# andimarafioti/faster-qwen3-tts

Measured on AMD Instinct MI355X. Metric: real-time factor (audio s / wall s), Qwen3-TTS-12Hz-0.6B voice-clone streaming chunk_size=8; p50 TTFA in ttfa_ms_p50, higher is better.
Workload: dtype bf16

## Files before the change

faster-qwen3-tts_amd/csrc/decode_kernels.cuh:

```cuda
#pragma once
#include "fq3_common.cuh"

namespace fq3 {

enum { PRO_PLAIN = 0, PRO_NORM = 1, PRO_COMBINE = 2 };
enum { EPI_STORE = 0, EPI_RESIDUAL = 1, EPI_SWIGLU = 2 };

constexpr int kHeadDim = 128;
constexpr int kKeysPerTile = 64;
constexpr int kMaxWorkers = 8;
constexpr int kPartStride = kHeadDim + 4;


struct GemvArgs {
    const void* W; int N; int K;
    const void* x;
    const void* norm_w; float eps;
    const void* bias;
    void* y;
    const void* res;
    void* xn_out;
    int up_off;
    const float* part; int n_part; int rep;
    const void* x2; void* y2; const void* res2; size_t part_stride2;
// ... 371 lines not shown
        for (int w = 0; w < 4; ++w) {
            const float ww = __expf(wm[w][h] - M);
            num = fmaf(ww, wo[w][h][d], num);
            den = fmaf(ww, wl[w][h], den);
        }
        float* p = a.part + (((size_t)g * kMaxWorkers + s) * REP + h) * kPartStride;
        p[d] = num;
        if (d == 0) { p[HD] = M; p[HD + 1] = den; }
    }
}

template <typename T, int REP, bool PAGED>
__global__ __launch_bounds__(256) void attn_decode_kernel(AttnArgs a) { attn_decode_body<T, REP, PAGED>(a); }

template <typename T>
__device__ __forceinline__ void attn_pred_body(const AttnArgs& a, int head) {
    constexpr int HD = kHeadDim;
    const int g = head / a.rep, hh = head - g * a.rep;
    const int lane = threadIdx.x & 63, sub = lane >> 4, c = lane & 15;
    const int pos = a.pos_imm;
    const T* qkv = reinterpret_cast<const T*>(a.qkv);
    const int q_dim = a.n_kv * a.rep * HD, kv_dim = a.n_kv * HD;
    T* kc = reinterpret_cast<T*>(a.kcache) + (size_t)g * a.max_seq * HD;
    T* vc = reinterpret_cast<T*>(a.vcache) + (size_t)g * a.max_seq * HD;
    Raw8<T> qraw, knraw, vnraw, qwraw, kwraw, kr[4], vr[4];
    ldraw<false>(qraw, qkv + (size_t)head * HD + c * 8);
    ldraw<false>(knraw, qkv + q_dim + (size_t)g * HD + c * 8);
    ldraw<false>(vnraw, qkv + q_dim + kv_dim + (size_t)g * HD + c * 8);
    ldraw<false>(qwraw, reinterpret_cast<const T*>(a.q_norm_w) + c * 8);
    ldraw<false>(kwraw, reinterpret_cast<const T*>(a.k_norm_w) + c * 8);
    const f32x4 cs0 = *reinterpret_cast<const f32x4*>(a.cos_row + ((c * 8) & 63)), cs1 = *reinterpret_cast<const f32x4*>(a.cos_row + ((c * 8 + 4) & 63));
    const f32x4 sn0 = *reinterpret_cast<const f32x4*>(a.sin_row + ((c * 8) & 63)), sn1 = *reinterpret_cast<const f32x4*>(a.sin_row + ((c * 8 + 4) & 63));
#pragma unroll
    for (int i = 0; i < 4; ++i) {
        int key = i * 4 + sub;
        key = key < a.max_seq ? key : a.max_seq - 1;
        ldraw<false>(kr[i], kc + (size_t)key * HD + c * 8);
        ldraw<false>(vr[i], vc + (size_t)key * HD + c * 8);
    }
    __builtin_amdgcn_sched_barrier(0);
    const float sgn = c < 8 ? -1.f : 1.f;
    const float cs[8] = {cs0.x, cs0.y, cs0.z, cs0.w, cs1.x, cs1.y, cs1.z, cs1.w};
    const float sn[8] = {sgn * sn0.x, sgn * sn0.y, sgn * sn0.z, sgn * sn0.w, sgn * sn1.x, sgn * sn1.y, sgn * sn1.z, sgn * sn1.w};
    auto norm_rope = [&](const Raw8<T>& raw, const Raw8<T>& wraw, float (&out)[8]) {
        float x[8], w[8];
        unpack(raw, x); unpack(wraw, w);
        float ss = 0.f;
#pragma unroll
        for (int i = 0; i < 8; ++i) ss = fmaf(x[i], x[i], ss);
        ss = row16_sum(ss);
        const float rs = 1.0f / sqrtf(ss / (float)HD + a.eps);
#pragma unroll
        for (int i = 0; i < 8; i += 2) {
            float u = x[i] * rs, v = x[i + 1] * rs;
            DT<T>::rnd2(u, v);
            u *= w[i]; v *= w[i + 1];
            DT<T>::rnd2(u, v);
            x[i] = u; x[i + 1] = v;
        }
#pragma unroll
        for (int i = 0; i < 8; i += 2) {
            float a0 = x[i] * cs[i], a1 = x[i + 1] * cs[i + 1];
            float b0 = row16_xor8(x[i]) * sn[i], b1 = row16_xor8(x[i + 1]) * sn[i + 1];
            DT<T>::rnd2(a0, a1); DT<T>::rnd2(b0, b1);
            float r0 = a0 + b0, r1 = a1 + b1;
            DT<T>::rnd2(r0, r1);
            out[i] = r0; out[i + 1] = r1;
        }
    };
    float qr[8], knew[8], vnew[8];
    norm_rope(qraw, qwraw, qr);
    norm_rope(knraw, kwraw, knew);
    unpack(vnraw, vnew);
    if (hh == 0 && sub == 0) {
        DT<T>::st8(kc + (size_t)pos * HD + c * 8, knew);
        DT<T>::st8(vc + (size_t)pos * HD + c * 8, vnew);
    }
    float sc[5];
#pragma unroll
    for (int i = 0; i < 4; ++i) {
        float kf[8], s = 0.f;
        unpack(kr[i], kf);
#pragma unroll
        for (int d = 0; d < 8; ++d) s = fmaf(qr[d], kf[d], s);
// ... 18 lines not shown
    for (int i = 0; i < 4; ++i) {
        float vf[8];
        if (!(i * 4 + sub < pos)) zero(vr[i]);
        unpack(vr[i], vf);
#pragma unroll
        for (int d = 0; d < 8; ++d) o[d] = fmaf(p[i], vf[d], o[d]);
    }
    const float inv = 1.0f / lsum;
#pragma unroll
    for (int d = 0; d < 8; ++d) o[d] = xrow_sum(o[d]) * inv;
    if (sub == 0) DT<T>::st8(reinterpret_cast<T*>(a.out) + (size_t)head * HD + c * 8, o);
}

template <typename T>
__device__ __forceinline__ void attn_pred_body(const AttnArgs& a) { attn_pred_body<T>(a, (int)blockIdx.x); }

template <typename T, int REP>
__device__ __forceinline__ void attn_pred_group_body(const AttnArgs& a, int g) {
    constexpr int HD = kHeadDim;
    const int lane = threadIdx.x & 63, sub = lane >> 4, c = lane & 15;
    const int pos = a.pos_imm;
    const T* qkv = reinterpret_cast<const T*>(a.qkv);
    const int q_dim = a.n_kv * REP * HD, kv_dim = a.n_kv * HD;
    T* kc = reinterpret_cast<T*>(a.kcache) + (size_t)g * a.max_seq * HD;
    T* vc = reinterpret_cast<T*>(a.vcache) + (size_t)g * a.max_seq * HD;
    Raw8<T> qraw[REP], knraw, vnraw, qwraw, kwraw, kr[4], vr[4];
#pragma unroll
    for (int h = 0; h < REP; ++h) ldraw<false>(qraw[h], qkv + (size_t)(g * REP + h) * HD + c * 8);
    ldraw<false>(knraw, qkv + q_dim + (size_t)g * HD + c * 8);
    ldraw<false>(vnraw, qkv + q_dim + kv_dim + (size_t)g * HD + c * 8);
    ldraw<false>(qwraw, reinterpret_cast<const T*>(a.q_norm_w) + c * 8);
    ldraw<false>(kwraw, reinterpret_cast<const T*>(a.k_norm_w) + c * 8);
    const f32x4 cs0 = *reinterpret_cast<const f32x4*>(a.cos_row + ((c * 8) & 63)), cs1 = *reinterpret_cast<const f32x4*>(a.cos_row + ((c * 8 + 4) & 63));
    const f32x4 sn0 = *reinterpret_cast<const f32x4*>(a.sin_row + ((c * 8) & 63)), sn1 = *reinterpret_cast<const f32x4*>(a.sin_row + ((c * 8 + 4) & 63));
#pragma unroll
    for (int i = 0; i < 4; ++i) {
        int key = i * 4 + sub;
        key = key < pos ? key : 0;
        ldraw<false>(kr[i], kc + (size_t)key * HD + c * 8);
        ldraw<false>(vr[i], vc + (size_t)key * HD + c * 8);
    }
    __builtin_amdgcn_sched_barrier(0);
    const float sgn = c < 8 ? -1.f : 1.f;
    const float cs[8] = {cs0.x, cs0.y, cs0.z, cs0.w, cs1.x, cs1.y, cs1.z, cs1.w};
    const float sn[8] = {sgn * sn0.x, sgn * sn0.y, sgn * sn0.z, sgn * sn0.w, sgn * sn1.x, sgn * sn1.y, sgn * sn1.z, sgn * sn1.w};
    auto norm_rope = [&](const Raw8<T>& raw, const Raw8<T>& wraw, float (&out)[8]) {
        float x[8], w[8];
        unpack(raw, x); unpack(wraw, w);
        float ss = 0.f;
#pragma unroll
        for (int i = 0; i < 8; ++i) ss = fmaf(x[i], x[i], ss);
        ss = row16_sum(ss);
        const float rs = 1.0f / sqrtf(ss / (float)HD + a.eps);
#pragma unroll
        for (int i = 0; i < 8; i += 2) {
            float u = x[i] * rs, v = x[i + 1] * rs;
            DT<T>::rnd2(u, v);
            u *= w[i]; v *= w[i + 1];
            DT<T>::rnd2(u, v);
            x[i] = u; x[i + 1] = v;
        }
#pragma unroll
        for (int i = 0; i < 8; i += 2) {
            float a0 = x[i] * cs[i], a1 = x[i + 1] * cs[i + 1];
            float b0 = row16_xor8(x[i]) * sn[i], b1 = row16_xor8(x[i + 1]) * sn[i + 1];
            DT<T>::rnd2(a0, a1); DT<T>::rnd2(b0, b1);
            float r0 = a0 + b0, r1 = a1 + b1;
            DT<T>::rnd2(r0, r1);
            out[i] = r0; out[i + 1] = r1;
        }
    };
    float knew[8], vnew[8];
    norm_rope(knraw, kwraw, knew);
    unpack(vnraw, vnew);
    if (sub == 0) {
        DT<T>::st8(kc + (size_t)pos * HD + c * 8, knew);
        DT<T>::st8(vc + (size_t)pos * HD + c * 8, vnew);
    }
    float kf[4][8], vf[4][8];
#pragma unroll
    for (int i = 0; i < 4; ++i) {
        unpack(kr[i], kf[i]);
        if (!(i * 4 + sub < pos)) zero(vr[i]);
        unpack(vr[i], vf[i]);
    }
#pragma unroll
    for (int h = 0; h < REP; ++h) {
        float qr[8];
        norm_rope(qraw[h], qwraw, qr);
        float sc[5];
#pragma unroll
        for (int i = 0; i < 4; ++i) {
            float s = 0.f;
#pragma unroll
            for (int d = 0; d < 8; ++d) s = fmaf(qr[d], kf[i][d], s);
            s = row16_sum(s);
            sc[i] = (i * 4 + sub < pos) ? s * a.scale : -INFINITY;
        }
        {
            float s = 0.f;
#pragma unroll
            for (int d = 0; d < 8; ++d) s = fmaf(qr[d], knew[d], s);
            s = row16_sum(s);
            sc[4] = sub == 0 ? s * a.scale : -INFINITY;
        }
        const float mx = wave_max(fmaxf(fmaxf(fmaxf(sc[0], sc[1]), fmaxf(sc[2], sc[3])), sc[4]));
        float p[5], lsum = 0.f, o[8];
#pragma unroll
        for (int i = 0; i < 5; ++i) { p[i] = __expf(sc[i] - mx); lsum += p[i]; }
        lsum = wave_sum(lsum) * (1.0f / 16.0f);
#pragma unroll
        for (int d = 0; d < 8; ++d) o[d] = p[4] * vnew[d];
#pragma unroll
        for (int i = 0; i < 4; ++i)
#pragma unroll
            for (int d = 0; d < 8; ++d) o[d] = fmaf(p[i], vf[i][d], o[d]);
        const float inv = 1.0f / lsum;
#pragma unroll
        for (int d = 0; d < 8; ++d) o[d] = xrow_sum(o[d]) * inv;
        if (sub == 0) DT<T>::st8(reinterpret_cast<T*>(a.out) + (size_t)(g * REP + h) * HD + c * 8, o);
    }
}

template <typename T>
__global__ __launch_bounds__(64) void attn_pred_kernel(AttnArgs a) { attn_pred_body<T>(a); }

template <typename T>
__global__ __launch_bounds__(256) void rmsnorm_kernel(const T* x, const T* w, T* y, int K, float eps) {
    __shared__ float red[8];
    float ss = 0.f;
    for (int e = threadIdx.x; e < K; e += 256) { const float v = DT<T>::ld(x + e); ss = fmaf(v, v, ss); }
    ss = block_sum<4>(ss, red);
    const float rs = 1.0f / sqrtf(ss / (float)K + eps);
    for (int e = threadIdx.x; e < K; e += 256)
        DT<T>::st(y + e, DT<T>::ld(w + e) * DT<T>::rnd(DT<T>::ld(x + e) * rs));
}

template <typename T>
__global__ void copy_kernel(T* dst, const T* src, int n) {
    const int i = blockIdx.x * blockDim.x + threadIdx.x;
// ... 97 lines not shown
```

faster-qwen3-tts_amd/csrc/fq3_api.hip:

```cpp
#define FQ3_SKINNY_EXTERN
#include "fq3_ctx.h"
#include "sampler.cuh"
#include "sampler_wave.cuh"
#include "skinny_gemm.cuh"

#include <cstdio>
#include <cstdlib>
#include <cstring>
#include <map>
#include <string>
#include <type_traits>
#include <vector>

using namespace fq3;

static thread_local std::string g_err;
static int fail(int code, const std::string& m) { g_err = m; return code; }
int fq3_fail_(int code, const std::string& m) { return fail(code, m); }
#define HIPCHK(x) do { hipError_t e_ = (x); if (e_ != hipSuccess) return fail(FQ3_EHIP, std::string(#x) + ": " + hipGetErrorString(e_)); } while (0)

extern "C" const char* fq3_last_error(void) { return g_err.c_str(); }
extern "C" void fq3_set_error_(const char* msg) { g_err = msg ? msg : ""; }
extern "C" int fq3_abi_version(void) { return FQ3_ABI_VERSION; }

// ... 217 lines not shown
}

extern "C" int fq3_set_option(fq3_ctx* c, const char* key, int value) {
    if (!c || !key) return fail(FQ3_EINVAL, "null argument");
    const std::string k(key);
    if (k == "weight_nt") c->opt_nt = value;
    else if (k == "pred_m2") c->opt_m2 = value;
    else if (k == "pred_attn") c->opt_pred_attn = value;
    else if (k == "rows_per_wave_max") c->opt_rmax = value;
    else if (k == "prefill_mode") c->prefill_mode = value;
    else if (k == "flash_prefill") c->opt_flash_prefill = value;
    else if (k == "flash_small") c->opt_flash_small = value;
    else if (k == "swiglu_tile") c->opt_swiglu_tile = value;
    else if (k == "packed_weights") c->opt_packed = value;
    else if (k == "skinny_gemm") c->opt_no_skinny = !value;
    else return fail(FQ3_EINVAL, "unknown option: " + k);
    fq3_graph_reset(c);
    return FQ3_OK;
}

extern "C" int fq3_graph_reset(fq3_ctx* c) {
    if (!c) return fail(FQ3_EINVAL, "null ctx");
    if (c->exec) { (void)hipGraphExecDestroy(c->exec); c->exec = nullptr; }
    if (c->graph) { (void)hipGraphDestroy(c->graph); c->graph = nullptr; }
    return FQ3_OK;
}

namespace {
struct PackedEntry { void* p; int refs; int N, K; };
std::mutex g_packed_mu;
// ... 44 lines not shown
            if (int r = take(l.o, d.hidden, qd, 0)) return r;
            if (int r = take(l.gate_up, 2 * d.inter, d.hidden, 1)) return r;
            if (int r = take(l.gate_up, 2 * d.inter, d.hidden, 0)) return r;
            if (int r = take(l.down, d.hidden, d.inter, 0)) return r;
        }
        return FQ3_OK;
    };
    if (int r = stack(c->tl, c->cfg.talker)) return r;
    if (int r = stack(c->pl, c->cfg.predictor)) return r;
    for (const fq3_layer_weights& l : c->tl) if (int r = take(l.gate_up, 2 * c->cfg.talker.inter, c->cfg.talker.hidden, 2)) return r;
    if (int r = take(c->wt.codec_head, c->cfg.talker.vocab, c->cfg.talker.hidden, 0)) return r;
    for (const void* h : c->lmh) if (int r = take(h, c->cfg.predictor.vocab, c->cfg.predictor.hidden, 0)) return r;
    return FQ3_OK;
}

extern "C" int fq3_ctx_destroy(fq3_ctx* c) {
    if (!c) return FQ3_OK;
    (void)hipDeviceSynchronize();
    fq3_graph_reset(c);
    packed_release_all(c);
    if (c->cap_stream) (void)hipStreamDestroy(c->cap_stream);
    if (fq3_kv_pool* p = c->tk.pool) {
        (void)fq3_kv_release(c, 0);
        bool last;
        { std::lock_guard<std::mutex> lk(p->mu); last = --p->users == 0; }
        if (p->is_private && last) pool_free_(p);
    }
    for (void* p : c->allocs) (void)hipFree(p);
    delete c;
    return FQ3_OK;
}

extern "C" int fq3_bind_weights(fq3_ctx* c, const fq3_weight_table* w) {
    if (!c || !w) return fail(FQ3_EINVAL, "null argument");
    const int G = c->cfg.num_code_groups;
// ... 4 lines not shown
    if (c->cfg.has_projection && !w->proj_w) return fail(FQ3_EINVAL, "has_projection set but proj_w is null");
    if (w->talker_rope_len < c->cfg.max_seq_len || w->pred_rope_len < G + 1)
        return fail(FQ3_EINVAL, "rope tables shorter than the caches");
    c->wt = *w;
    c->tl.assign(w->talker_layers, w->talker_layers + c->cfg.talker.n_layers);
    c->pl.assign(w->predictor_layers, w->predictor_layers + c->cfg.predictor.n_layers);
    c->pemb.assign(w->predictor_embeddings, w->predictor_embeddings + (G - 1));
    c->lmh.assign(w->lm_heads, w->lm_heads + (G - 1));
    for (auto& l : c->tl) if (!l.qkv || !l.o || !l.gate_up || !l.down || !l.input_norm || !l.post_norm || !l.q_norm || !l.k_norm)
        return fail(FQ3_EINVAL, "talker layer has null weights");
    for (auto& l : c->pl) if (!l.qkv || !l.o || !l.gate_up || !l.down || !l.input_norm || !l.post_norm || !l.q_norm || !l.k_norm)
        return fail(FQ3_EINVAL, "predictor layer has null weights");
    HIPCHK(hipMemcpy(c->d_pemb, c->pemb.data(), (G - 1) * sizeof(void*), hipMemcpyHostToDevice));
    (void)hipDeviceSynchronize();
    packed_release_all(c);
    if (int r = packed_acquire_all(c)) { packed_release_all(c); return r; }
    c->bound = true;
    fq3_graph_reset(c);
    return FQ3_OK;
}

static thread_local int g_rmax = 2;
template <typename T, int NCH, int PRO, int EPI, bool NT, int M = 1>
static void launch_gemv_n(const GemvArgs& a, hipStream_t s) {
    const int rmax = g_rmax;
    int R = (a.N + 1023) / 1024;
    if (R > MaxRows<NCH, EPI>::v) R = MaxRows<NCH, EPI>::v;
    if (rmax > 0 && R > rmax) R = rmax;
    if (R < 1) R = 1;
    const int grid = (a.N + 4 * R - 1) / (4 * R);
    const size_t shm = PRO == PRO_COMBINE ? (size_t)M * a.K * sizeof(float) : 0;
// ... 37 lines not shown
    return nt ? launch_gemv_t<float, PRO, EPI, true>(a, s) : launch_gemv_t<float, PRO, EPI, false>(a, s);
}

template <typename T, bool PAGED>
static void launch_attn_p(const AttnArgs& a, int rep, int workers, hipStream_t s) {
    dim3 grid(a.n_kv, workers);
    if (rep == 1) hipLaunchKernelGGL((attn_decode_kernel<T, 1, PAGED>), grid, dim3(256), 0, s, a);
    else if (rep == 2) hipLaunchKernelGGL((attn_decode_kernel<T, 2, PAGED>), grid, dim3(256), 0, s, a);
    else hipLaunchKernelGGL((attn_decode_kernel<T, 4, PAGED>), grid, dim3(256), 0, s, a);
}
template <typename T>
static void launch_attn_t(const AttnArgs& a, int rep, int workers, hipStream_t s) {
    if (a.table) launch_attn_p<T, true>(a, rep, workers, s); else launch_attn_p<T, false>(a, rep, workers, s);
}

struct StepSrc { const void* x0; const int* pos_ptr; int pos_imm; bool kv_only_tail = false; };

static int run_stack(fq3_ctx* c, bool talker, const StepSrc& src, hipStream_t s) {
    const fq3_stack_dims& d = talker ? c->cfg.talker : c->cfg.predictor;
    const std::vector<fq3_layer_weights>& L = talker ? c->tl : c->pl;
    StackBufs& kv = talker ? c->tk : c->pk;
    const int rep = d.n_heads / d.n_kv_heads;
    const int q_dim = d.n_heads * kHeadDim, kv_dim = d.n_kv_heads * kHeadDim;
    const bool nt = c->opt_nt == 2 || (c->opt_nt == 1 && talker);
    const float *cos_row, *sin_row;
    if (src.pos_ptr) { cos_row = c->rope_now; sin_row = c->rope_now + 64; }
    else {
        const int rl = talker ? c->wt.talker_rope_len : c->wt.pred_rope_len;
        int rp = src.pos_imm + (talker ? c->rope_delta : 0);
        rp = rp < 0 ? 0 : (rp >= rl ? rl - 1 : rp);
        cos_row = (talker ? c->wt.talker_cos : c->wt.pred_cos) + (size_t)rp * 64;
        sin_row = (talker ? c->wt.talker_sin : c->wt.pred_sin) + (size_t)rp * 64;
    }
    for (int i = 0; i < d.n_layers; ++i) {
        const fq3_layer_weights& w = L[i];
        const void* xin = i == 0 ? src.x0 : c->h;
        GemvArgs g{};
        g.eps = d.rms_eps;
        g.W = w.qkv; g.N = q_dim + 2 * kv_dim; g.K = d.hidden; g.x = xin;
        g.norm_w = w.input_norm; g.y = c->qkv;
        if (int r = launch_gemv<PRO_NORM, EPI_STORE>(c, g, nt, s)) return r;
        const bool tail_skip = src.kv_only_tail && i == d.n_layers - 1;
        GemvArgs o{};
        o.W = w.o; o.N = d.hidden; o.K = q_dim; o.y = c->h; o.res = xin; o.rep = rep;
        AttnArgs a{};
        a.qkv = c->qkv; a.q_norm_w = w.q_norm; a.k_norm_w = w.k_norm; a.eps = d.rms_eps;
        a.cos_row = cos_row; a.sin_row = sin_row;
        a.kcache = kv.k[i]; a.vcache = kv.v[i]; a.max_seq = kv.max_seq;
        a.table = kv.d_table; a.blk_stride = kv.pool ? (int)kv.pool->blk_elems : 0;
        a.pos_ptr = src.pos_ptr; a.pos_imm = src.pos_imm;
        a.done_ptr = src.pos_ptr ? &c->st->done : nullptr;
        a.n_pad = talker ? c->n_pad : 0;
        a.n_kv = d.n_kv_heads; a.part = c->part;
        a.scale = 1.0f / sqrtf((float)kHeadDim);
        a.rep = rep; a.out = c->attn_out;
        const bool pred_attn = c->opt_pred_attn && !talker && !src.pos_ptr && src.pos_imm <= 16;
        if (pred_attn) {
            if (c->cfg.dtype == FQ3_BF16) hipLaunchKernelGGL((attn_pred_kernel<bf16_t>), dim3(d.n_heads), dim3(64), 0, s, a);
            else hipLaunchKernelGGL((attn_pred_kernel<float>), dim3(d.n_heads), dim3(64), 0, s, a);
            if (tail_skip) break;
            o.x = c->attn_out;
            if (int r = launch_gemv<PRO_PLAIN, EPI_RESIDUAL>(c, o, nt, s)) return r;
        } else {
            if (c->cfg.dtype == FQ3_BF16) launch_attn_t<bf16_t>(a, rep, kv.workers, s);
            else launch_attn_t<float>(a, rep, kv.workers, s);
            if (tail_skip) break;
            o.part = c->part; o.n_part = kv.workers;
            if (int r = launch_gemv<PRO_COMBINE, EPI_RESIDUAL>(c, o, nt, s)) return r;
        }
        GemvArgs m{};
        m.eps = d.rms_eps; m.W = w.gate_up; m.N = d.inter; m.K = d.hidden; m.x = c->h;
        m.norm_w = w.post_norm; m.y = c->act; m.up_off = d.inter;
        if (int r = launch_gemv<PRO_NORM, EPI_SWIGLU>(c, m, nt, s)) return r;
// ... 301 lines not shown
}

template <typename T>
static void launch_sample_pred(const DecodeState* st, const T* lg, int V, int cb, const SampleCfg& cfg, const T* nz,
                               int* codes, int G, int64_t* out64, const T* next_emb, T* next_in, int H, bool wave,
                               const TeacherForcing* tf, hipStream_t s) {
    if (wave) dispatch_nc(V, [&](auto nc) {
        constexpr int NC = decltype(nc)::value;
        hipLaunchKernelGGL((sample_pred_wave_kernel<T, NC>), dim3(1), dim3(256), 0, s, st, lg, V, cb, cfg, nz, codes, G,
                           out64, next_emb, next_in, H, tf);
    });
    else hipLaunchKernelGGL((sample_pred_kernel<T>), dim3(1), dim3(256), 0, s, st, lg, V, cb, cfg, nz, codes, G, out64,
                            next_emb, next_in, H, tf);
}
template <typename T>
static void launch_sample_talker(DecodeState* st, const T* lg, int V, const unsigned char* seen, int G, bool wave,
                                 const TeacherForcing* tf, hipStream_t s) {
    if (wave) dispatch_nc(V, [&](auto nc) {
        constexpr int NC = decltype(nc)::value;
        hipLaunchKernelGGL((sample_talker_wave_kernel<T, NC>), dim3(1), dim3(256), 0, s, st, lg, V, seen, G, tf);
    });
    else hipLaunchKernelGGL((sample_talker_kernel<T>), dim3(1), dim3(256), 0, s, st, lg, V, seen, G, tf);
}
template <typename T>
static void launch_sample_api(fq3_ctx* c, const T* lg, int V, const SampleCfg& cfg, const int64_t* history, int n_hist,
                              const T* noise, int64_t* out, hipStream_t s) {
    if (cfg.top_p >= 1.0f) {
        const unsigned char* seen = nullptr;
        if (n_hist > 0) {
            hipLaunchKernelGGL(build_seen_kernel, dim3(1), dim3(256), 0, s, history, n_hist, c->seen_api, V);
// ... 57 lines not shown

extern "C" int fq3_set_predictor_sampling(fq3_ctx* c, const fq3_sampling* s) {
    if (!c || !s) return fail(FQ3_EINVAL, "null argument");
    if (s->do_sample && !(s->temperature > 0.f)) return fail(FQ3_EINVAL, "temperature must be > 0");
    if ((s->top_p >= 1.0f) != (c->pred_sampling.top_p >= 1.0f)) fq3_graph_reset(c);
    c->pred_sampling = *s;
    return FQ3_OK;
}

template <typename T>
static int predictor_passes_t(fq3_ctx* c, const DecodeState* st_dev, const void* pred_input, const void* noise_imm,
                              int64_t* out64, void* out_logits, hipStream_t s) {
    const fq3_stack_dims &p = c->cfg.predictor, &t = c->cfg.talker;
    const int G = c->cfg.num_code_groups, Vp = p.vocab, Ht = t.hidden;
    SampleCfg scfg = to_cfg(c->pred_sampling);
    for (int pass = 0; pass < G; ++pass) {
        const void* hsrc = c->h;
        if (pass == 0 && c->opt_m2) {
            const T* xa = (const T*)pred_input;
            const T* xb = (const T*)pred_input + Ht;
            if (c->cfg.has_projection) {
                GemvArgs g{};
                g.W = c->wt.proj_w; g.bias = c->wt.proj_b; g.N = p.hidden; g.K = Ht; g.x = xa; g.x2 = xb; g.y = c->pred_x; g.y2 = c->pred_x2;
                if (int r = launch_gemv2<PRO_PLAIN, EPI_STORE>(c, g, s)) return r;
                xa = (const T*)c->pred_x; xb = (const T*)c->pred_x2;
            }
            if (int r = run_predictor_pair(c, xa, xb, s)) return r;
            pass = 1;
            hsrc = c->h2;
        } else {
        const T* x_talker = pass < 2 ? (const T*)pred_input + (size_t)pass * Ht : (const T*)c->pred_next;
        const void* x0 = x_talker;
        if (c->cfg.has_projection) {
            GemvArgs g{};
            g.W = c->wt.proj_w; g.bias = c->wt.proj_b; g.N = p.hidden; g.K = Ht; g.x = x_talker; g.y = c->pred_x;
            if (int r = launch_gemv<PRO_PLAIN, EPI_STORE>(c, g, false, s)) return r;
            x0 = c->pred_x;
        }
        StepSrc src{x0, nullptr, pass};
        src.kv_only_tail = pass == 0;
        if (int r = run_stack(c, false, src, s)) return r;
        }
        if (pass == 0) continue;
        const int cb = pass - 1;
        T* lg = out_logits ? (T*)out_logits + (size_t)cb * Vp : (T*)c->plogits + (size_t)cb * Vp;
        GemvArgs hgm{};
        hgm.eps = p.rms_eps; hgm.W = c->lmh[cb]; hgm.N = Vp; hgm.K = p.hidden; hgm.x = hsrc;
        hgm.norm_w = c->wt.predictor_final_norm; hgm.y = lg;
        if (int r = launch_gemv<PRO_NORM, EPI_STORE>(c, hgm, false, s)) return r;
        const T* nz = noise_imm ? (const T*)noise_imm + (size_t)cb * Vp : nullptr;
        const T* next_emb = cb + 1 < G - 1 ? (const T*)c->pemb[cb] : nullptr;
        launch_sample_pred<T>(st_dev, (const T*)lg, Vp, cb, scfg, nz, st_dev ? c->codes : nullptr, G, out64, next_emb,
                              (T*)c->pred_next, Ht, c->pred_sampling.top_p >= 1.0f, st_dev ? c->tf : nullptr, s);
    }
    return 0;
}

extern "C" int fq3_predictor_loop(fq3_ctx* c, const void* pred_input, const void* noise, int64_t* out_ids,
                                  void* out_logits, void* stream) {
    NEED_BOUND(c);
    if (!pred_input || !out_ids) return fail(FQ3_EINVAL, "null argument");
    if (c->pred_sampling.do_sample && !noise) return fail(FQ3_EINVAL, "predictor sampling enabled but no noise given");
    hipStream_t s = (hipStream_t)stream;
    int r = c->cfg.dtype == FQ3_BF16 ? predictor_passes_t<bf16_t>(c, nullptr, pred_input, noise, out_ids, out_logits, s)
                                     : predictor_passes_t<float>(c, nullptr, pred_input, noise, out_ids, out_logits, s);
    if (r) return r;
    LAUNCH_CHECK();
    return FQ3_OK;
// ... 146 lines not shown
```

faster-qwen3-tts_amd/csrc/fq3_ctx.h:

```cpp
#pragma once
#include "../../include/fq3hip.h"
#include "decode_kernels.cuh"
#include <hip/hip_runtime.h>
#include <mutex>
#include <string>
#include <utility>
#include <vector>

struct fq3_kv_pool {
    int dtype = 0, esz = 2, n_layers = 0, n_kv = 0, n_blocks = 0;
    size_t blk_elems = 0;
    std::vector<void*> k, v;
    std::vector<int> free_list;
    std::mutex mu;
    int in_use_high = 0;
    int users = 0;
    bool is_private = false;
};

struct StackBufs {
    std::vector<void*> k, v;
    int max_seq = 0, workers = 1;
    fq3_kv_pool* pool = nullptr;
    int* d_table = nullptr;
// ... 21 lines not shown
    fq3::DecodeState* st = nullptr;
    fq3::TeacherForcing* tf = nullptr;
    unsigned char* seen = nullptr;
    int* codes = nullptr;
    int64_t* ids64 = nullptr;
    int n_pad = 0, rope_delta = 0;
    int opt_nt = 1;
    int opt_m2 = 1;
    int opt_pred_attn = 1;
    int opt_rmax = 2;
    int opt_flash_prefill = 1;
    int opt_flash_small = 1;
    int opt_swiglu_tile = 1;
    int opt_packed = 1;
    std::vector<std::pair<const void*, int>> packed_refs;
    int opt_no_skinny = 0;
    int prefill_mode = 0;
    bool talker_wave = true;
    fq3_sampling pred_sampling{0.9f, 50, 1.0f, 1, 1.0f};
    hipGraph_t graph = nullptr;
    hipGraphExec_t exec = nullptr;
    hipStream_t cap_stream = nullptr;
    std::vector<void*> allocs;
    fq3_prompt_weights pw{};
    bool pw_bound = false;
    void *pw_x = nullptr, *pw_h = nullptr;
    int pw_cap = 0;
    void *pf_x = nullptr, *pf_xn = nullptr, *pf_qkv = nullptr, *pf_att = nullptr, *pf_gu = nullptr, *pf_act = nullptr, *pf_ws = nullptr;
};

// ... 14 lines not shown
```

faster-qwen3-tts_amd/csrc/sampler_wave.cuh:

```cuda
#pragma once
#include "sampler.cuh"

namespace fq3 {

__device__ __forceinline__ ArgMax wave_argmax(ArgMax a) {
    ArgMax r;
    r.v = wave_max(a.v);
    r.i = wave_min_i32(a.v == r.v ? a.i : 0x7fffffff);
    return r;
}

struct BlkSmem { int cnt[2][4]; float f[4]; float av[4]; int ai[4]; };

__device__ __forceinline__ float blk_max4(float v, BlkSmem& sm) {
    v = wave_max(v);
    __syncthreads();
    if ((threadIdx.x & 63) == 0) sm.f[threadIdx.x >> 6] = v;
    __syncthreads();
    return fmaxf(fmaxf(sm.f[0], sm.f[1]), fmaxf(sm.f[2], sm.f[3]));
}
__device__ __forceinline__ float blk_sum4(float v, BlkSmem& sm) {
    v = wave_sum(v);
    __syncthreads();
    if ((threadIdx.x & 63) == 0) sm.f[threadIdx.x >> 6] = v;
// ... 137 lines not shown
        float f[8];
        unpack(xraw[j], f);
#pragma unroll
        for (int i = 0; i < 8; ++i) {
            const int id = j * 2048 + threadIdx.x * 8 + i;
            if (id < V) big.vals[id] = f[i];
        }
    }
    __syncthreads();
    const int tok = sample_core<T>(big, V, c, seen, noise);
    __syncthreads();
    return tok;
}

template <typename T, int NC, bool NUCLEUS = false>
__device__ __forceinline__ void sample_pred_wave_body(const DecodeState* st, const T* logits, int V, int cb,
                                                      const SampleCfg& c_imm, const T* noise_imm, int* codes, int G,
                                                      int64_t* out64, const T* next_emb, T* next_in, int H, const TeacherForcing* tf = nullptr) {
    __shared__ BlkSmem sm;
    Raw8<T> xraw[NC];
    issue_logits<T, NC>(xraw, logits, V);
    SampleCfg c = c_imm;
    const T* noise = noise_imm;
    int frame = 0;
    if (st) {
        if (st->done) return;
        c.temperature = st->p_temperature; c.top_k = st->p_top_k; c.top_p = st->p_top_p; c.do_sample = st->p_do_sample;
        frame = st->frame;
        if (st->pred_noise)
            noise = gptr(reinterpret_cast<const T*>(st->pred_noise)) + ((size_t)(frame % st->noise_frames) * (G - 1) + cb) * V;
    }
    int tok;
    if constexpr (NUCLEUS) {
        __shared__ SampleSmem big;
// ... 7 lines not shown
        if (codes) codes[(size_t)frame * G + 1 + cb] = tok;
        if (out64) out64[cb] = tok;
    }
    if (next_emb) {
        const T* src = next_emb + (size_t)tok * H;
        for (int e = threadIdx.x * 8; e < H; e += 256 * 8) {
            Raw8<T> r; ldraw<false>(r, src + e);
            if (sizeof(T) == 2) *reinterpret_cast<u32x4*>(reinterpret_cast<char*>(next_in) + (size_t)e * 2) = *reinterpret_cast<u32x4*>(&r);
            else { float f[8]; unpack(r, f);
#pragma unroll
                   for (int i = 0; i < 8; ++i) DT<T>::st(next_in + e + i, f[i]); }
        }
    }
}

template <typename T, int NC>
__global__ __launch_bounds__(256) void sample_pred_wave_kernel(const DecodeState* st, const T* logits, int V, int cb,
                                                              SampleCfg c_imm, const T* noise_imm, int* codes, int G,
                                                              int64_t* out64, const T* next_emb, T* next_in, int H, const TeacherForcing* tf) {
    sample_pred_wave_body<T, NC>(st, logits, V, cb, c_imm, noise_imm, codes, G, out64, next_emb, next_in, H, tf);
}

template <typename T, int NC, bool NUCLEUS = false>
__device__ __forceinline__ void sample_talker_wave_body(DecodeState* st, const T* logits, int V, const unsigned char* seen, int G,
                                                        const TeacherForcing* tf = nullptr) {
    __shared__ BlkSmem sm;
    Raw8<T> xraw[NC];
    issue_logits<T, NC>(xraw, logits, V);
    if (st->done) return;
    SampleCfg c;
    c.temperature = st->t_temperature; c.top_k = st->t_top_k; c.top_p = st->t_top_p; c.do_sample = st->t_do_sample;
    c.rep_penalty = st->t_rep_penalty;
    c.sup_lo = st->sup_lo; c.sup_hi = st->sup_hi; c.keep_id = st->eos_id;
    const int frame = st->frame;
    c.sup_extra = (frame + 1 < st->min_new) ? st->eos_id : -1;
// ... 21 lines not shown
```

Before: 36.85.

## Precompute per-token predictor layer-0 QKV table and fuse layer-0 attention into sampler

For each predictor codebook embedding, the layer-0 input-norm, QKV projection, head norm and RoPE are precomputed once at bind time into a per-token table shared across contexts. During decode, extra waves in the sampling kernel mirror the sampler's barrier sequence to learn the chosen token. They then read that token's precomputed QKV row, write the KV cache and run layer-0 attention, so run_stack skips layer-0 QKV GEMV and attention for later passes. This adds a large table allocation and build cost, and the barrier-mirroring code is tightly coupled to the sampler's sync structure, which is fragile.

```diff
diff --git a/faster-qwen3-tts_amd/csrc/decode_kernels.cuh b/faster-qwen3-tts_amd/csrc/decode_kernels.cuh
--- a/faster-qwen3-tts_amd/csrc/decode_kernels.cuh
+++ b/faster-qwen3-tts_amd/csrc/decode_kernels.cuh
@@ -409,6 +409,35 @@
 __global__ __launch_bounds__(256) void attn_decode_kernel(AttnArgs a) { attn_decode_body<T, REP, PAGED>(a); }
 
 template <typename T>
+__device__ __forceinline__ void head_norm_rope(const Raw8<T>& raw, const Raw8<T>& wraw, const float (&cs)[8], const float (&sn)[8],
+                                               float eps, float (&out)[8]) {
+    float x[8], w[8];
+    unpack(raw, x); unpack(wraw, w);
+    float ss = 0.f;
+#pragma unroll
+    for (int i = 0; i < 8; ++i) ss = fmaf(x[i], x[i], ss);
+    ss = row16_sum(ss);
+    const float rs = 1.0f / sqrtf(ss / (float)kHeadDim + eps);
+#pragma unroll
+    for (int i = 0; i < 8; i += 2) {
+        float u = x[i] * rs, v = x[i + 1] * rs;
+        DT<T>::rnd2(u, v);
+        u *= w[i]; v *= w[i + 1];
+        DT<T>::rnd2(u, v);
+        x[i] = u; x[i + 1] = v;
+    }
+#pragma unroll
+    for (int i = 0; i < 8; i += 2) {
+        float a0 = x[i] * cs[i], a1 = x[i + 1] * cs[i + 1];
+        float b0 = row16_xor8(x[i]) * sn[i], b1 = row16_xor8(x[i + 1]) * sn[i + 1];
+        DT<T>::rnd2(a0, a1); DT<T>::rnd2(b0, b1);
+        float r0 = a0 + b0, r1 = a1 + b1;
+        DT<T>::rnd2(r0, r1);
+        out[i] = r0; out[i + 1] = r1;
+    }
+}
+
+template <typename T>
 __device__ __forceinline__ void attn_pred_body(const AttnArgs& a, int head) {
     constexpr int HD = kHeadDim;
     const int g = head / a.rep, hh = head - g * a.rep;
@@ -437,32 +466,7 @@
     const float sgn = c < 8 ? -1.f : 1.f;
     const float cs[8] = {cs0.x, cs0.y, cs0.z, cs0.w, cs1.x, cs1.y, cs1.z, cs1.w};
     const float sn[8] = {sgn * sn0.x, sgn * sn0.y, sgn * sn0.z, sgn * sn0.w, sgn * sn1.x, sgn * sn1.y, sgn * sn1.z, sgn * sn1.w};
-    auto norm_rope = [&](const Raw8<T>& raw, const Raw8<T>& wraw, float (&out)[8]) {
-        float x[8], w[8];
-        unpack(raw, x); unpack(wraw, w);
-        float ss = 0.f;
-#pragma unroll
-        for (int i = 0; i < 8; ++i) ss = fmaf(x[i], x[i], ss);
-        ss = row16_sum(ss);
-        const float rs = 1.0f / sqrtf(ss / (float)HD + a.eps);
-#pragma unroll
-        for (int i = 0; i < 8; i += 2) {
-            float u = x[i] * rs, v = x[i + 1] * rs;
-            DT<T>::rnd2(u, v);
-            u *= w[i]; v *= w[i + 1];
-            DT<T>::rnd2(u, v);
-            x[i] = u; x[i + 1] = v;
-        }
-#pragma unroll
-        for (int i = 0; i < 8; i += 2) {
-            float a0 = x[i] * cs[i], a1 = x[i + 1] * cs[i + 1];
-            float b0 = row16_xor8(x[i]) * sn[i], b1 = row16_xor8(x[i + 1]) * sn[i + 1];
-            DT<T>::rnd2(a0, a1); DT<T>::rnd2(b0, b1);
-            float r0 = a0 + b0, r1 = a1 + b1;
-            DT<T>::rnd2(r0, r1);
-            out[i] = r0; out[i + 1] = r1;
-        }
-    };
+    auto norm_rope = [&](const Raw8<T>& raw, const Raw8<T>& wraw, float (&out)[8]) { head_norm_rope<T>(raw, wraw, cs, sn, a.eps, out); };
     float qr[8], knew[8], vnew[8];
     norm_rope(qraw, qwraw, qr);
     norm_rope(knraw, kwraw, knew);
@@ -511,6 +515,56 @@
 
 template <typename T>
 __device__ __forceinline__ void attn_pred_body(const AttnArgs& a) { attn_pred_body<T>(a, (int)blockIdx.x); }
+
+template <typename T, int REP, typename QF>
+__device__ __forceinline__ void pred_group_attend(QF&& qof, const Raw8<T> (&kr)[4], Raw8<T> (&vr)[4], const float (&knew)[8],
+                                                  const float (&vnew)[8], int pos, float scale, T* out) {
+    constexpr int HD = kHeadDim;
+    const int lane = threadIdx.x & 63, sub = lane >> 4, c = lane & 15;
+    float kf[4][8], vf[4][8];
+#pragma unroll
+    for (int i = 0; i < 4; ++i) {
+        unpack(kr[i], kf[i]);
+        if (!(i * 4 + sub < pos)) zero(vr[i]);
+        unpack(vr[i], vf[i]);
+    }
+#pragma unroll
+    for (int h = 0; h < REP; ++h) {
+        float qr[8];
+        qof(h, qr);
+        float sc[5];
+#pragma unroll
+        for (int i = 0; i < 4; ++i) {
+            float s = 0.f;
+#pragma unroll
+            for (int d = 0; d < 8; ++d) s = fmaf(qr[d], kf[i][d], s);
+            s = row16_sum(s);
+            sc[i] = (i * 4 + sub < pos) ? s * scale : -INFINITY;
+        }
+        {
+            float s = 0.f;
+#pragma unroll
+            for (int d = 0; d < 8; ++d) s = fmaf(qr[d], knew[d], s);
+            s = row16_sum(s);
+            sc[4] = sub == 0 ? s * scale : -INFINITY;
+        }
+        const float mx = wave_max(fmaxf(fmaxf(fmaxf(sc[0], sc[1]), fmaxf(sc[2], sc[3])), sc[4]));
+        float p[5], lsum = 0.f, o[8];
+#pragma unroll
+        for (int i = 0; i < 5; ++i) { p[i] = __expf(sc[i] - mx); lsum += p[i]; }
+        lsum = wave_sum(lsum) * (1.0f / 16.0f);
+#pragma unroll
+        for (int d = 0; d < 8; ++d) o[d] = p[4] * vnew[d];
+#pragma unroll
+        for (int i = 0; i < 4; ++i)
+#pragma unroll
+            for (int d = 0; d < 8; ++d) o[d] = fmaf(p[i], vf[i][d], o[d]);
+        const float inv = 1.0f / lsum;
+#pragma unroll
+        for (int d = 0; d < 8; ++d) o[d] = xrow_sum(o[d]) * inv;
+        if (sub == 0) DT<T>::st8(out + (size_t)h * HD + c * 8, o);
+    }
+}
 
 template <typename T, int REP>
 __device__ __forceinline__ void attn_pred_group_body(const AttnArgs& a, int g) {
@@ -541,32 +595,7 @@
     const float sgn = c < 8 ? -1.f : 1.f;
     const float cs[8] = {cs0.x, cs0.y, cs0.z, cs0.w, cs1.x, cs1.y, cs1.z, cs1.w};
     const float sn[8] = {sgn * sn0.x, sgn * sn0.y, sgn * sn0.z, sgn * sn0.w, sgn * sn1.x, sgn * sn1.y, sgn * sn1.z, sgn * sn1.w};
-    auto norm_rope = [&](const Raw8<T>& raw, const Raw8<T>& wraw, float (&out)[8]) {
-        float x[8], w[8];
-        unpack(raw, x); unpack(wraw, w);
-        float ss = 0.f;
-#pragma unroll
-        for (int i = 0; i < 8; ++i) ss = fmaf(x[i], x[i], ss);
-        ss = row16_sum(ss);
-        const float rs = 1.0f / sqrtf(ss / (float)HD + a.eps);
-#pragma unroll
-        for (int i = 0; i < 8; i += 2) {
-            float u = x[i] * rs, v = x[i + 1] * rs;
-            DT<T>::rnd2(u, v);
-            u *= w[i]; v *= w[i + 1];
-            DT<T>::rnd2(u, v);
-            x[i] = u; x[i + 1] = v;
-        }
-#pragma unroll
-        for (int i = 0; i < 8; i += 2) {
-            float a0 = x[i] * cs[i], a1 = x[i + 1] * cs[i + 1];
-            float b0 = row16_xor8(x[i]) * sn[i], b1 = row16_xor8(x[i + 1]) * sn[i + 1];
-            DT<T>::rnd2(a0, a1); DT<T>::rnd2(b0, b1);
-            float r0 = a0 + b0, r1 = a1 + b1;
-            DT<T>::rnd2(r0, r1);
-            out[i] = r0; out[i + 1] = r1;
-        }
-    };
+    auto norm_rope = [&](const Raw8<T>& raw, const Raw8<T>& wraw, float (&out)[8]) { head_norm_rope<T>(raw, wraw, cs, sn, a.eps, out); };
     float knew[8], vnew[8];
     norm_rope(knraw, kwraw, knew);
     unpack(vnraw, vnew);
@@ -574,53 +603,49 @@
         DT<T>::st8(kc + (size_t)pos * HD + c * 8, knew);
         DT<T>::st8(vc + (size_t)pos * HD + c * 8, vnew);
     }
-    float kf[4][8], vf[4][8];
-#pragma unroll
-    for (int i = 0; i < 4; ++i) {
-        unpack(kr[i], kf[i]);
-        if (!(i * 4 + sub < pos)) zero(vr[i]);
-        unpack(vr[i], vf[i]);
-    }
-#pragma unroll
-    for (int h = 0; h < REP; ++h) {
-        float qr[8];
-        norm_rope(qraw[h], qwraw, qr);
-        float sc[5];
-#pragma unroll
-        for (int i = 0; i < 4; ++i) {
-            float s = 0.f;
-#pragma unroll
-            for (int d = 0; d < 8; ++d) s = fmaf(qr[d], kf[i][d], s);
-            s = row16_sum(s);
-            sc[i] = (i * 4 + sub < pos) ? s * a.scale : -INFINITY;
-        }
-        {
-            float s = 0.f;
-#pragma unroll
-            for (int d = 0; d < 8; ++d) s = fmaf(qr[d], knew[d], s);
-            s = row16_sum(s);
-            sc[4] = sub == 0 ? s * a.scale : -INFINITY;
-        }
-        const float mx = wave_max(fmaxf(fmaxf(fmaxf(sc[0], sc[1]), fmaxf(sc[2], sc[3])), sc[4]));
-        float p[5], lsum = 0.f, o[8];
-#pragma unroll
-        for (int i = 0; i < 5; ++i) { p[i] = __expf(sc[i] - mx); lsum += p[i]; }
-        lsum = wave_sum(lsum) * (1.0f / 16.0f);
-#pragma unroll
-        for (int d = 0; d < 8; ++d) o[d] = p[4] * vnew[d];
-#pragma unroll
-        for (int i = 0; i < 4; ++i)
-#pragma unroll
-            for (int d = 0; d < 8; ++d) o[d] = fmaf(p[i], vf[i][d], o[d]);
-        const float inv = 1.0f / lsum;
-#pragma unroll
-        for (int d = 0; d < 8; ++d) o[d] = xrow_sum(o[d]) * inv;
-        if (sub == 0) DT<T>::st8(reinterpret_cast<T*>(a.out) + (size_t)(g * REP + h) * HD + c * 8, o);
-    }
+    pred_group_attend<T, REP>([&](int h, float (&qr)[8]) { norm_rope(qraw[h], qwraw, qr); }, kr, vr, knew, vnew, pos, a.scale,
+                              reinterpret_cast<T*>(a.out) + (size_t)g * REP * HD);
 }
 
 template <typename T>
 __global__ __launch_bounds__(64) void attn_pred_kernel(AttnArgs a) { attn_pred_body<T>(a); }
+
+template <typename T, int NCH, int R, int TPB>
+__global__ __launch_bounds__(256) void gemv_norm_tokens_kernel(GemvArgs a, int n_tok, size_t x_stride, size_t y_stride) {
+    const T* x0 = reinterpret_cast<const T*>(a.x);
+    T* y0 = reinterpret_cast<T*>(a.y);
+#pragma unroll 1
+    for (int i = 0; i < TPB; ++i) {
+        const int t = blockIdx.y * TPB + i;
+        if (t >= n_tok) break;
+        a.x = x0 + (size_t)t * x_stride;
+        a.y = y0 + (size_t)t * y_stride;
+        gemv_body<T, NCH, PRO_NORM, EPI_STORE, false, 1, R>(a);
+    }
+}
+
+template <typename T>
+__global__ __launch_bounds__(256) void head_norm_rope_rows_kernel(T* rows, int n_tok, int row_len, int n_q, int n_k, const T* q_norm_w,
+                                                                  const T* k_norm_w, const float* cos_row, const float* sin_row, float eps) {
+    const int lane = threadIdx.x & 63, sub = lane >> 4, c = lane & 15;
+    const int nh = n_q + n_k;
+    const long total = (long)n_tok * nh;
+    const long r = (long)blockIdx.x * 16 + (threadIdx.x >> 6) * 4 + sub;
+    const long rc = r < total ? r : total - 1;
+    const int tok = (int)(rc / nh), hv = (int)(rc - (long)tok * nh);
+    T* p = rows + (size_t)tok * row_len + (size_t)hv * kHeadDim + c * 8;
+    Raw8<T> raw, wraw;
+    ldraw<false>(raw, p);
+    ldraw<false>(wraw, (hv < n_q ? q_norm_w : k_norm_w) + c * 8);
+    const f32x4 cs0 = *reinterpret_cast<const f32x4*>(cos_row + ((c * 8) & 63)), cs1 = *reinterpret_cast<const f32x4*>(cos_row + ((c * 8 + 4) & 63));
+    const f32x4 sn0 = *reinterpret_cast<const f32x4*>(sin_row + ((c * 8) & 63)), sn1 = *reinterpret_cast<const f32x4*>(sin_row + ((c * 8 + 4) & 63));
+    const float sgn = c < 8 ? -1.f : 1.f;
+    const float cs[8] = {cs0.x, cs0.y, cs0.z, cs0.w, cs1.x, cs1.y, cs1.z, cs1.w};
+    const float sn[8] = {sgn * sn0.x, sgn * sn0.y, sgn * sn0.z, sgn * sn0.w, sgn * sn1.x, sgn * sn1.y, sgn * sn1.z, sgn * sn1.w};
+    float o[8];
+    head_norm_rope<T>(raw, wraw, cs, sn, eps, o);
+    if (r < total) DT<T>::st8(p, o);
+}
 
 template <typename T>
 __global__ __launch_bounds__(256) void rmsnorm_kernel(const T* x, const T* w, T* y, int K, float eps) {
diff --git a/faster-qwen3-tts_amd/csrc/fq3_api.hip b/faster-qwen3-tts_amd/csrc/fq3_api.hip
--- a/faster-qwen3-tts_amd/csrc/fq3_api.hip
+++ b/faster-qwen3-tts_amd/csrc/fq3_api.hip
@@ -255,6 +255,7 @@
     else if (k == "swiglu_tile") c->opt_swiglu_tile = value;
     else if (k == "packed_weights") c->opt_packed = value;
     else if (k == "skinny_gemm") c->opt_no_skinny = !value;
+    else if (k == "pred_tok_table") c->opt_tok_table = value;
     else return fail(FQ3_EINVAL, "unknown option: " + k);
     fq3_graph_reset(c);
     return FQ3_OK;
@@ -329,11 +330,85 @@
     return FQ3_OK;
 }
 
+namespace {
+struct TokTable { void* p; int refs; };
+std::mutex g_ttab_mu;
+std::map<std::vector<const void*>, TokTable> g_ttab;
+}
+static bool tok_table_supported(const fq3_ctx* c) {
+    const fq3_stack_dims& d = c->cfg.predictor;
+    const int rep = d.n_heads / d.n_kv_heads, G = c->cfg.num_code_groups;
+    return c->cfg.dtype == FQ3_BF16 && !c->cfg.has_projection && d.n_kv_heads <= 8 && (rep == 1 || rep == 2 || rep == 4) &&
+           G >= 3 && G <= 16 && d.hidden <= 2048;
+}
+static std::vector<const void*> tok_table_key(const fq3_ctx* c) {
+    const fq3_stack_dims& d = c->cfg.predictor;
+    const fq3_layer_weights& w = c->pl[0];
+    std::vector<const void*> k = {w.qkv, w.input_norm, w.q_norm, w.k_norm, c->wt.pred_cos, c->wt.pred_sin,
+                                  reinterpret_cast<const void*>((intptr_t)d.vocab), reinterpret_cast<const void*>((intptr_t)d.hidden),
+                                  reinterpret_cast<const void*>((intptr_t)d.n_heads), reinterpret_cast<const void*>((intptr_t)d.n_kv_heads)};
+    for (int cb = 0; cb + 2 < c->cfg.num_code_groups; ++cb) k.push_back(c->pemb[cb]);
+    return k;
+}
+template <int NCH>
+static void tok_table_gemv(const GemvArgs& g, int n_tok, int H, int row) {
+    constexpr int R = 2, TPB = 16;
+    const dim3 grid((g.N + 4 * R - 1) / (4 * R), (n_tok + TPB - 1) / TPB);
+    hipLaunchKernelGGL((gemv_norm_tokens_kernel<bf16_t, NCH, R, TPB>), grid, dim3(256), 0, nullptr, g, n_tok, (size_t)H, (size_t)row);
+}
+static int tok_table_build(fq3_ctx* c, void** out) {
+    const fq3_stack_dims& d = c->cfg.predictor;
+    const int Vp = d.vocab, H = d.hidden, n_tab = c->cfg.num_code_groups - 2;
+    const int q_dim = d.n_heads * kHeadDim, kv_dim = d.n_kv_heads * kHeadDim, row = q_dim + 2 * kv_dim;
+    const fq3_layer_weights& w = c->pl[0];
+    void* p = nullptr;
+    if (hipMalloc(&p, (size_t)n_tab * Vp * row * sizeof(bf16_t)) != hipSuccess) { (void)hipGetLastError(); return FQ3_ENOMEM; }
+    for (int cb = 0; cb < n_tab; ++cb) {
+        bf16_t* y = reinterpret_cast<bf16_t*>(p) + (size_t)cb * Vp * row;
+        GemvArgs g{};
+        g.eps = d.rms_eps; g.W = w.qkv; g.N = row; g.K = H; g.x = c->pemb[cb]; g.norm_w = w.input_norm; g.y = y;
+        const int need = (H + 511) / 512;
+        if (need <= 1) tok_table_gemv<1>(g, Vp, H, row);
+        else if (need <= 2) tok_table_gemv<2>(g, Vp, H, row);
+        else tok_table_gemv<4>(g, Vp, H, row);
+        const int rp = std::min(cb + 2, c->wt.pred_rope_len - 1);
+        const long heads = (long)Vp * (d.n_heads + d.n_kv_heads);
+        hipLaunchKernelGGL((head_norm_rope_rows_kernel<bf16_t>), dim3((unsigned)((heads + 15) / 16)), dim3(256), 0, nullptr, y, Vp, row,
+                           d.n_heads, d.n_kv_heads, (const bf16_t*)w.q_norm, (const bf16_t*)w.k_norm, c->wt.pred_cos + (size_t)rp * 64,
+                           c->wt.pred_sin + (size_t)rp * 64, d.rms_eps);
+    }
+    if (hipGetLastError() != hipSuccess || hipStreamSynchronize(nullptr) != hipSuccess) { (void)hipFree(p); return FQ3_EHIP; }
+    *out = p;
+    return FQ3_OK;
+}
+static void tok_table_release(fq3_ctx* c) {
+    if (!c->ptab) return;
+    std::lock_guard<std::mutex> lk(g_ttab_mu);
+    for (auto it = g_ttab.begin(); it != g_ttab.end(); ++it)
+        if (it->second.p == c->ptab) {
+            if (--it->second.refs <= 0) { (void)hipFree(it->second.p); g_ttab.erase(it); }
+            break;
+        }
+    c->ptab = nullptr;
+}
+static void tok_table_acquire(fq3_ctx* c) {
+    if (!tok_table_supported(c)) return;
+    const std::vector<const void*> key = tok_table_key(c);
+    std::lock_guard<std::mutex> lk(g_ttab_mu);
+    auto it = g_ttab.find(key);
+    if (it != g_ttab.end()) { ++it->second.refs; c->ptab = it->second.p; return; }
+    void* p = nullptr;
+    if (tok_table_build(c, &p) != FQ3_OK) return;
+    g_ttab[key] = TokTable{p, 1};
+    c->ptab = p;
+}
+
 extern "C" int fq3_ctx_destroy(fq3_ctx* c) {
     if (!c) return FQ3_OK;
     (void)hipDeviceSynchronize();
     fq3_graph_reset(c);
     packed_release_all(c);
+    tok_table_release(c);
     if (c->cap_stream) (void)hipStreamDestroy(c->cap_stream);
     if (fq3_kv_pool* p = c->tk.pool) {
         (void)fq3_kv_release(c, 0);
@@ -368,7 +443,9 @@
     HIPCHK(hipMemcpy(c->d_pemb, c->pemb.data(), (G - 1) * sizeof(void*), hipMemcpyHostToDevice));
     (void)hipDeviceSynchronize();
     packed_release_all(c);
+    tok_table_release(c);
     if (int r = packed_acquire_all(c)) { packed_release_all(c); return r; }
+    tok_table_acquire(c);
     c->bound = true;
     fq3_graph_reset(c);
     return FQ3_OK;
@@ -436,7 +513,7 @@
     if (a.table) launch_attn_p<T, true>(a, rep, workers, s); else launch_attn_p<T, false>(a, rep, workers, s);
 }
 
-struct StepSrc { const void* x0; const int* pos_ptr; int pos_imm; bool kv_only_tail = false; };
+struct StepSrc { const void* x0; const int* pos_ptr; int pos_imm; bool kv_only_tail = false; bool l0_attn_done = false; };
 
 static int run_stack(fq3_ctx* c, bool talker, const StepSrc& src, hipStream_t s) {
     const fq3_stack_dims& d = talker ? c->cfg.talker : c->cfg.predictor;
@@ -457,11 +534,13 @@
     for (int i = 0; i < d.n_layers; ++i) {
         const fq3_layer_weights& w = L[i];
         const void* xin = i == 0 ? src.x0 : c->h;
+        const bool l0_done = i == 0 && src.l0_attn_done;
         GemvArgs g{};
         g.eps = d.rms_eps;
         g.W = w.qkv; g.N = q_dim + 2 * kv_dim; g.K = d.hidden; g.x = xin;
         g.norm_w = w.input_norm; g.y = c->qkv;
-        if (int r = launch_gemv<PRO_NORM, EPI_STORE>(c, g, nt, s)) return r;
+        if (!l0_done)
+            if (int r = launch_gemv<PRO_NORM, EPI_STORE>(c, g, nt, s)) return r;
         const bool tail_skip = src.kv_only_tail && i == d.n_layers - 1;
         GemvArgs o{};
         o.W = w.o; o.N = d.hidden; o.K = q_dim; o.y = c->h; o.res = xin; o.rep = rep;
@@ -477,8 +556,10 @@
         a.scale = 1.0f / sqrtf((float)kHeadDim);
         a.rep = rep; a.out = c->attn_out;
         const bool pred_attn = c->opt_pred_attn && !talker && !src.pos_ptr && src.pos_imm <= 16;
+        if (l0_done && !pred_attn) return fq3_fail_(FQ3_EINVAL, "run_stack: layer 0 from the token table needs the one-wave predictor attention");
         if (pred_attn) {
-            if (c->cfg.dtype == FQ3_BF16) hipLaunchKernelGGL((attn_pred_kernel<bf16_t>), dim3(d.n_heads), dim3(64), 0, s, a);
+            if (l0_done) {}
+            else if (c->cfg.dtype == FQ3_BF16) hipLaunchKernelGGL((attn_pred_kernel<bf16_t>), dim3(d.n_heads), dim3(64), 0, s, a);
             else hipLaunchKernelGGL((attn_pred_kernel<float>), dim3(d.n_heads), dim3(64), 0, s, a);
             if (tail_skip) break;
             o.x = c->attn_out;
@@ -810,6 +891,20 @@
                             next_emb, next_in, H, tf);
 }
 template <typename T>
+static void launch_sample_pred_l0(const DecodeState* st, const T* lg, int V, int cb, const SampleCfg& cfg, const T* nz, int* codes, int G,
+                                  int64_t* out64, const T* next_emb, T* next_in, int H, const TeacherForcing* tf, const PredL0Args& l0,
+                                  int rep, hipStream_t s) {
+    if constexpr (std::is_same<T, bf16_t>::value) {
+        const dim3 block(256 + 64 * l0.n_kv);
+        dispatch_nc(V, [&](auto nc) {
+            constexpr int NC = decltype(nc)::value;
+            if (rep == 1) hipLaunchKernelGGL((sample_pred_attn_kernel<T, NC, 1>), dim3(1), block, 0, s, st, lg, V, cb, cfg, nz, codes, G, out64, next_emb, next_in, H, tf, l0);
+            else if (rep == 2) hipLaunchKernelGGL((sample_pred_attn_kernel<T, NC, 2>), dim3(1), block, 0, s, st, lg, V, cb, cfg, nz, codes, G, out64, next_emb, next_in, H, tf, l0);
+            else hipLaunchKernelGGL((sample_pred_attn_kernel<T, NC, 4>), dim3(1), block, 0, s, st, lg, V, cb, cfg, nz, codes, G, out64, next_emb, next_in, H, tf, l0);
+        });
+    }
+}
+template <typename T>
 static void launch_sample_talker(DecodeState* st, const T* lg, int V, const unsigned char* seen, int G, bool wave,
                                  const TeacherForcing* tf, hipStream_t s) {
     if (wave) dispatch_nc(V, [&](auto nc) {
@@ -897,6 +992,9 @@
     const fq3_stack_dims &p = c->cfg.predictor, &t = c->cfg.talker;
     const int G = c->cfg.num_code_groups, Vp = p.vocab, Ht = t.hidden;
     SampleCfg scfg = to_cfg(c->pred_sampling);
+    const bool wave = c->pred_sampling.top_p >= 1.0f;
+    const bool tab = std::is_same<T, bf16_t>::value && c->ptab && c->opt_tok_table && c->opt_pred_attn && wave;
+    const int q_dim = p.n_heads * kHeadDim, kv_dim = p.n_kv_heads * kHeadDim;
     for (int pass = 0; pass < G; ++pass) {
         const void* hsrc = c->h;
         if (pass == 0 && c->opt_m2) {
@@ -922,6 +1020,7 @@
         }
         StepSrc src{x0, nullptr, pass};
         src.kv_only_tail = pass == 0;
+        src.l0_attn_done = tab && pass >= 2;
         if (int r = run_stack(c, false, src, s)) return r;
         }
         if (pass == 0) continue;
@@ -933,8 +1032,18 @@
         if (int r = launch_gemv<PRO_NORM, EPI_STORE>(c, hgm, false, s)) return r;
         const T* nz = noise_imm ? (const T*)noise_imm + (size_t)cb * Vp : nullptr;
         const T* next_emb = cb + 1 < G - 1 ? (const T*)c->pemb[cb] : nullptr;
-        launch_sample_pred<T>(st_dev, (const T*)lg, Vp, cb, scfg, nz, st_dev ? c->codes : nullptr, G, out64, next_emb,
-                              (T*)c->pred_next, Ht, c->pred_sampling.top_p >= 1.0f, st_dev ? c->tf : nullptr, s);
+        if (tab && next_emb) {
+            PredL0Args l0{};
+            l0.row_len = q_dim + 2 * kv_dim;
+            l0.tab = (const T*)c->ptab + (size_t)cb * Vp * l0.row_len;
+            l0.kcache = c->pk.k[0]; l0.vcache = c->pk.v[0]; l0.max_seq = c->pk.max_seq;
+            l0.out = c->attn_out; l0.n_kv = p.n_kv_heads; l0.pos = pass + 1; l0.scale = 1.0f / sqrtf((float)kHeadDim);
+            launch_sample_pred_l0<T>(st_dev, (const T*)lg, Vp, cb, scfg, nz, st_dev ? c->codes : nullptr, G, out64, next_emb,
+                                     (T*)c->pred_next, Ht, st_dev ? c->tf : nullptr, l0, p.n_heads / p.n_kv_heads, s);
+        } else {
+            launch_sample_pred<T>(st_dev, (const T*)lg, Vp, cb, scfg, nz, st_dev ? c->codes : nullptr, G, out64, next_emb,
+                                  (T*)c->pred_next, Ht, wave, st_dev ? c->tf : nullptr, s);
+        }
     }
     return 0;
 }
diff --git a/faster-qwen3-tts_amd/csrc/fq3_ctx.h b/faster-qwen3-tts_amd/csrc/fq3_ctx.h
--- a/faster-qwen3-tts_amd/csrc/fq3_ctx.h
+++ b/faster-qwen3-tts_amd/csrc/fq3_ctx.h
@@ -59,6 +59,8 @@
     int opt_swiglu_tile = 1;
     int opt_packed = 1;
     std::vector<std::pair<const void*, int>> packed_refs;
+    int opt_tok_table = 1;
+    const void* ptab = nullptr;
     int opt_no_skinny = 0;
     int prefill_mode = 0;
     bool talker_wave = true;
diff --git a/faster-qwen3-tts_amd/csrc/sampler_wave.cuh b/faster-qwen3-tts_amd/csrc/sampler_wave.cuh
--- a/faster-qwen3-tts_amd/csrc/sampler_wave.cuh
+++ b/faster-qwen3-tts_amd/csrc/sampler_wave.cuh
@@ -175,10 +175,10 @@
 }
 
 template <typename T, int NC, bool NUCLEUS = false>
-__device__ __forceinline__ void sample_pred_wave_body(const DecodeState* st, const T* logits, int V, int cb,
+__device__ __forceinline__ void sample_pred_wave_impl(const DecodeState* st, const T* logits, int V, int cb,
                                                       const SampleCfg& c_imm, const T* noise_imm, int* codes, int G,
-                                                      int64_t* out64, const T* next_emb, T* next_in, int H, const TeacherForcing* tf = nullptr) {
-    __shared__ BlkSmem sm;
+                                                      int64_t* out64, const T* next_emb, T* next_in, int H, const TeacherForcing* tf,
+                                                      BlkSmem& sm) {
     Raw8<T> xraw[NC];
     issue_logits<T, NC>(xraw, logits, V);
     SampleCfg c = c_imm;
@@ -216,11 +216,104 @@
     }
 }
 
+template <typename T, int NC, bool NUCLEUS = false>
+__device__ __forceinline__ void sample_pred_wave_body(const DecodeState* st, const T* logits, int V, int cb,
+                                                      const SampleCfg& c_imm, const T* noise_imm, int* codes, int G,
+                                                      int64_t* out64, const T* next_emb, T* next_in, int H, const TeacherForcing* tf = nullptr) {
+    __shared__ BlkSmem sm;
+    sample_pred_wave_impl<T, NC, NUCLEUS>(st, logits, V, cb, c_imm, noise_imm, codes, G, out64, next_emb, next_in, H, tf, sm);
+}
+
 template <typename T, int NC>
 __global__ __launch_bounds__(256) void sample_pred_wave_kernel(const DecodeState* st, const T* logits, int V, int cb,
                                                               SampleCfg c_imm, const T* noise_imm, int* codes, int G,
                                                               int64_t* out64, const T* next_emb, T* next_in, int H, const TeacherForcing* tf) {
     sample_pred_wave_body<T, NC>(st, logits, V, cb, c_imm, noise_imm, codes, G, out64, next_emb, next_in, H, tf);
+}
+
+struct PredL0Args {
+    const void* tab; int row_len;
+    void* kcache; void* vcache; int max_seq;
+    void* out; int n_kv; int pos; float scale;
+};
+
+template <typename T>
+__device__ __forceinline__ int sample_wave_follow(int V, const SampleCfg& c, BlkSmem& sm) {
+    if (c.do_sample != 0) {
+        if (c.top_k > 0) {
+            const int kk = min(c.top_k, V);
+            constexpr int kLowBit = sizeof(T) == 2 ? 16 : 0;
+#pragma unroll 1
+            for (int bit = 31; bit >= kLowBit; --bit) {
+                __syncthreads();
+                const int* slot = sm.cnt[bit & 1];
+                const int tot = (slot[0] + slot[1]) + (slot[2] + slot[3]);
+                if (tot == kk) break;
+            }
+        }
+        __syncthreads(); __syncthreads();
+        __syncthreads(); __syncthreads();
+    }
+    __syncthreads(); __syncthreads();
+    ArgMax r; r.v = sm.av[0]; r.i = sm.ai[0];
+#pragma unroll
+    for (int i = 1; i < 4; ++i) { ArgMax b; b.v = sm.av[i]; b.i = sm.ai[i]; r = amax2(r, b); }
+    return r.i;
+}
+
+template <typename T, int REP>
+__device__ __forceinline__ void pred_l0_group_wave(const DecodeState* st, int V, int cb, const SampleCfg& c_imm, int G,
+                                                   const TeacherForcing* tf, const PredL0Args& l0, int g, BlkSmem& sm) {
+    constexpr int HD = kHeadDim;
+    const int lane = threadIdx.x & 63, sub = lane >> 4, c = lane & 15;
+    const int pos = l0.pos;
+    T* kc = reinterpret_cast<T*>(l0.kcache) + (size_t)g * l0.max_seq * HD;
+    T* vc = reinterpret_cast<T*>(l0.vcache) + (size_t)g * l0.max_seq * HD;
+    Raw8<T> kr[4], vr[4];
+#pragma unroll
+    for (int i = 0; i < 4; ++i) {
+        int key = i * 4 + sub;
+        key = key < pos ? key : 0;
+        ldraw<false>(kr[i], kc + (size_t)key * HD + c * 8);
+        ldraw<false>(vr[i], vc + (size_t)key * HD + c * 8);
+    }
+    SampleCfg cf = c_imm;
+    int frame = 0;
+    if (st) {
+        if (st->done) return;
+        cf.top_k = st->p_top_k; cf.do_sample = st->p_do_sample;
+        frame = st->frame;
+    }
+    int tok = sample_wave_follow<T>(V, cf, sm);
+    if (st) tok = forced_or(tf, frame * G + 1 + cb, tok);
+    tok = tok < 0 ? 0 : (tok < V ? tok : V - 1);
+    const T* row = reinterpret_cast<const T*>(l0.tab) + (size_t)tok * l0.row_len;
+    const int q_dim = l0.n_kv * REP * HD, kv_dim = l0.n_kv * HD;
+    Raw8<T> qraw[REP], knraw, vnraw;
+#pragma unroll
+    for (int h = 0; h < REP; ++h) ldraw<false>(qraw[h], row + (size_t)(g * REP + h) * HD + c * 8);
+    ldraw<false>(knraw, row + q_dim + (size_t)g * HD + c * 8);
+    ldraw<false>(vnraw, row + q_dim + kv_dim + (size_t)g * HD + c * 8);
+    float knew[8], vnew[8];
+    unpack(knraw, knew);
+    unpack(vnraw, vnew);
+    if (sub == 0) {
+        DT<T>::st8(kc + (size_t)pos * HD + c * 8, knew);
+        DT<T>::st8(vc + (size_t)pos * HD + c * 8, vnew);
+    }
+    pred_group_attend<T, REP>([&](int h, float (&qr)[8]) { unpack(qraw[h], qr); }, kr, vr, knew, vnew, pos, l0.scale,
+                              reinterpret_cast<T*>(l0.out) + (size_t)g * REP * HD);
+}
+
+template <typename T, int NC, int REP>
+__global__ __launch_bounds__(768) void sample_pred_attn_kernel(const DecodeState* st, const T* logits, int V, int cb,
+                                                               SampleCfg c_imm, const T* noise_imm, int* codes, int G,
+                                                               int64_t* out64, const T* next_emb, T* next_in, int H,
+                                                               const TeacherForcing* tf, PredL0Args l0) {
+    __shared__ BlkSmem sm;
+    const int wave = __builtin_amdgcn_readfirstlane(threadIdx.x >> 6);
+    if (wave < 4) sample_pred_wave_impl<T, NC>(st, logits, V, cb, c_imm, noise_imm, codes, G, out64, next_emb, next_in, H, tf, sm);
+    else pred_l0_group_wave<T, REP>(st, V, cb, c_imm, G, tf, l0, wave - 4, sm);
 }
 
 template <typename T, int NC, bool NUCLEUS = false>
```

New measurement: 37.77 (median of 6 runs). 2.5% higher.
